# xdslproject/ExaHyPE

Hardware: AMD Instinct MI355X
Metric: DoF-updates/sec, 3D Euler p=5 fused STP+volume+Riemann, 1/2/4/8 MI355X (higher is better)
Workload: dtype f64

## Files before the change

### exahype_amd/csrc/dg_inst.hip

```cpp
#include <cstdarg>
#include <cstdio>
#include "exa_dg_kernels.hpp"
#include "exa_dg_boundary.hpp"
#if EXA_DIM == 2
#include "exa_dg_fused.hpp"
#endif
#if EXA_DIM == 3
#include <algorithm>
#include <vector>
#include "exa_dg_reg.hpp"
#include "exa_dg_stream.hpp"
#include "exa_dg_m8.hpp"
#endif
#include "exa_launch.hpp"

#ifndef EXA_DIM
#error "compile with -DEXA_DIM=2|3 -DEXA_PDE_ID=0|1|2"
#endif

namespace exa {

#if EXA_PDE_ID >= 100
}
#include EXA_USER_PDE_HEADER
// ... 386 lines not shown
    void* step = static_cast<char*>(ops->dev) + StageA<DIM, N, PDE, cpb_of(N)>::STEP_OFF;
    hipLaunchKernelGGL((dg_step_ops_kernel<N>), dim3(1), dim3(64), 0, s, static_cast<const DgOps<N>*>(ops->dev), static_cast<DgStepOps<N>*>(step), dt);
    return step;
}

template <int N>
static int launch_a(const double* u_in, double* u_out, double* trace, long ncells, const CellBox* box, double dt,
                    const double* idx, int n_it, const DgOpsHost* ops, hipStream_t s, const RegFuse* fuse = nullptr) {
    if (box->nbox <= 0) return 0;
    const StageAChoice choice = stage_a_kind<N>(n_it, ops->stage_a_variant, fuse != nullptr);
    [[maybe_unused]] char* img = static_cast<char*>(ops->dev);
    [[maybe_unused]] hipError_t e = hipSuccess;
    switch (choice.kind) {
    case StageAKind::Refused:
        set_error("%s", choice.why);
        return -1;
    case StageAKind::Plain:
        if constexpr (has_plain<N>()) {
            using SP = StagePlain<DIM, N, PDE>;
            auto pk = dg_stage_a_plain_kernel<DIM, N, PDE>;
            static KernelSetup st;
            if (int rc = kernel_setup(st, reinterpret_cast<const void*>(pk), SP::LDS_BYTES, "stage_a", "plain")) return rc;
            hipLaunchKernelGGL(pk, dim3((unsigned)box->nbox), dim3(SP::NT), SP::LDS_BYTES, s, u_in, u_out, trace, ncells, *box, dt, idx[0], idx[1],
                               idx[2], n_it, pack_ops<N>(ops), plain_geo(ops, idx));
            e = hipGetLastError();
            if (e != hipSuccess) { set_error("stage_a (plain) launch (N %d): %s", N, hipGetErrorString(e)); return -2; }
            return 0;
        }
        break;
#if EXA_DIM == 3
    case StageAKind::M8:
        if constexpr (has_m8<N>()) {
            using SM = StageAM8<PDE>;
            auto mk = dg_stage_a_m8_kernel<PDE>;
            static KernelSetup st;
            if (int rc = kernel_setup(st, reinterpret_cast<const void*>(mk), SM::LDS_BYTES, "stage_a", "m8")) return rc;
            const long mwant = box->nbox < SCRATCH_BLOCKS ? box->nbox : SCRATCH_BLOCKS;
            const long mgrid = mwant - ops->stage_a_reserve > 1 ? mwant - ops->stage_a_reserve : 1;
            const void* step = enqueue_step_ops<N>(ops, dt, s);
            hipLaunchKernelGGL(mk, dim3((unsigned)mgrid), dim3(SM::NT), SM::LDS_BYTES, s, u_in, u_out, trace, ncells, *box, dt,
                               idx[0], idx[1], idx[2], n_it, ops->dev, step, reinterpret_cast<const int*>(img + OpsImage<N>::M8_TAB_OFF), plain_geo(ops, idx));
            e = hipGetLastError();
            if (e != hipSuccess) { set_error("stage_a (m8) launch: %s", hipGetErrorString(e)); return -2; }
            return 0;
        }
        break;
    case StageAKind::Stream:
        if constexpr (has_stream<N>()) {
            if (!ops->scratch) { set_error("stage_a: slab missing for N = %d", N); return -1; }
            using SS = StageAStream<N, PDE, 1, 1>;
            auto sk = dg_stage_a_stream_kernel<N, PDE, 1, 1>;
            static KernelSetup st;
            if (int rc = kernel_setup(st, reinterpret_cast<const void*>(sk), SS::LDS_BYTES, "stage_a", "stream")) return rc;
            const long grid = box->nbox < SCRATCH_BLOCKS ? box->nbox : SCRATCH_BLOCKS;
            hipLaunchKernelGGL(sk, dim3((unsigned)grid), dim3(SS::NT), SS::LDS_BYTES, s, u_in, u_out, trace, ncells, *box, dt,
                               idx[0], idx[1], idx[2], n_it, ops->dev, static_cast<double*>(ops->scratch));
            e = hipGetLastError();
            if (e != hipSuccess) { set_error("stage_a (stream) launch (N %d): %s", N, hipGetErrorString(e)); return -2; }
            return 0;
        }
        break;
    case StageAKind::Reg:
        if constexpr (has_reg<N>() && !needs_scratch<N>()) {
            constexpr int CPW = EXA_REG_CPW;
            using SR = StageAReg<N, PDE, CPW>;
            auto rk = dg_stage_a_reg_kernel<N, PDE, CPW, false>;
            if constexpr (!PDE_XT_NCP) {
                if (fuse) rk = dg_stage_a_reg_kernel<N, PDE, CPW, true>;
            }
            static KernelSetup st[2];
            long resident = 0;
            if (int rc = kernel_setup(st[fuse ? 1 : 0], reinterpret_cast<const void*>(rk), SR::LDS_BYTES, "stage_a", "reg", SR::NT * CPW, &resident)) return rc;
            const long rgrid = persistent_grid((box->nbox + CPW - 1) / CPW, resident, ops->stage_a_reserve);
            const void* step = enqueue_step_ops<N>(ops, dt, s);
            hipLaunchKernelGGL(rk, dim3((unsigned)rgrid), dim3(SR::NT * CPW), SR::LDS_BYTES, s, u_in, u_out, trace, ncells, *box, dt,
                               idx[0], idx[1], idx[2], n_it, ops->dev, reinterpret_cast<const int*>(img + OpsImage<N>::REG_TAB_OFF),
                               step, fuse ? *fuse : RegFuse{}, plain_geo(ops, idx));
            e = hipGetLastError();
            if (e != hipSuccess) { set_error("stage_a (reg) launch (N %d): %s", N, hipGetErrorString(e)); return -2; }
            return 0;
        }
        break;
#else
    case StageAKind::M8: case StageAKind::Stream: case StageAKind::Reg: break;
#endif
    case StageAKind::Single:
        if constexpr (!needs_scratch<N>()) {
            constexpr int NT1 = 256;
            constexpr int NNc = ipow(N, DIM);
            constexpr int CPB1 = (NT1 / NNc) > 0 ? NT1 / NNc : 1;
            const long nb1 = (box->nbox + CPB1 - 1) / CPB1;
            hipLaunchKernelGGL((dg_stage_a_single_kernel<DIM, N, PDE, CPB1, NT1>), dim3((unsigned)nb1), dim3(NT1), 0, s, u_in, u_out,
                               trace, ncells, *box, dt, idx[0], idx[1], idx[2], ops->dev);
            e = hipGetLastError();
            if (e != hipSuccess) { set_error("stage_a (single stage) launch (dim %d, N %d): %s", DIM, N, hipGetErrorString(e)); return -2; }
            return 0;
        }
        break;
    case StageAKind::Lds:
        if constexpr (!needs_scratch<N>()) {
            constexpr int CPB = cpb_of(N);
            using SA = StageA<DIM, N, PDE, CPB>;
            auto kern = dg_stage_a_kernel<DIM, N, PDE, CPB>;
            static KernelSetup st;
            long resident = 0;
            if (int rc = kernel_setup(st, reinterpret_cast<const void*>(kern), SA::LDS_BYTES, "stage_a", "", SA::NT, &resident)) return rc;
            const long grid = persistent_grid((box->nbox + CPB - 1) / CPB, resident, ops->stage_a_reserve);
            enqueue_step_ops<N>(ops, dt, s);
            hipLaunchKernelGGL(kern, dim3((unsigned)grid), dim3(SA::NT), SA::LDS_BYTES, s, u_in, u_out, trace, ncells, *box, dt,
                               idx[0], idx[1], idx[2], n_it, ops->dev);
            e = hipGetLastError();
            if (e != hipSuccess) { set_error("stage_a launch (dim %d, N %d): %s", DIM, N, hipGetErrorString(e)); return -2; }
            return 0;
        }
        break;
    }
    set_error("stage_a: the kernel selected for dim %d, N = %d (kind %d) is not built", DIM, N, (int)choice.kind);
    return -1;
}

template <int N> static size_t scratch_bytes_n() {
#if EXA_DIM == 3
    if constexpr (has_stream<N>()) return (size_t)SCRATCH_BLOCKS * StageAStream<N, PDE, 1, 1>::SLAB_D * sizeof(double);
#endif
    return 0;
}

#endif

template <int N>
static int launch_b(double* u, const double* trace, const StageBBox* box, long ncells, double dt, const double* idx,
                    const DgOpsHost* ops, hipStream_t s) {
    constexpr int NFc = ipow(N, DIM - 1);
    constexpr bool SHUFFLE = pow2ceil(NFc) == NFc && !PDE_XT_NCP;
    constexpr int PER = 2 * DIM * (SHUFFLE ? pow2ceil(NFc) : NFc);
    constexpr int CPB = PER >= 256 ? 1 : 256 / PER;
    constexpr int NT_B = SHUFFLE ? ((CPB * PER + 63) / 64) * 64 : 256;
    StageBArgs A;
    long nbox = 1;
    for (int d = 0; d < 3; d++) {
        A.nc[d] = box->nc[d];
        A.lo[d] = box->lo[d];
        A.nb[d] = box->nb[d];
        nbox *= box->nb[d];
    }
    for (int f = 0; f < 6; f++) A.ghost[f] = box->ghost[f];
    A.lam = box->lam;
    if (A.lam && pde_has_xt<PDE>::value) { set_error("stage B with the CFL scan: term sets whose eigenvalues see x, t take the scan with coordinates (exa_pde_eval_device_at)"); return -1; }
    if (nbox <= 0) return 0;
    {
        constexpr int TE = 1 << EXA_STAGE_B_TILE_SHIFT;
        A.tiled = DIM == 3 && box->nb[0] % TE == 0 && box->nb[1] % TE == 0 && box->nb[2] % TE == 0;
    }
    const long nblocks = (nbox + CPB - 1) / CPB;
    if constexpr (!pde_has_xt<PDE>::value) {
        if (A.lam) {
            if constexpr (SHUFFLE)
                hipLaunchKernelGGL((dg_stage_b_kernel<DIM, N, PDE, CPB, NT_B, true>), dim3((unsigned)nblocks), dim3(NT_B), 0, s, u, trace, A,
                                   ncells, nbox, dt, idx[0], idx[1], idx[2], pack_ops<N>(ops));
            else
                hipLaunchKernelGGL((dg_stage_b_dense_kernel<DIM, N, PDE, CPB, NT_B, true>), dim3((unsigned)nblocks), dim3(NT_B), 0, s, u, trace,
                                   A, ncells, nbox, dt, idx[0], idx[1], idx[2], pack_ops<N>(ops), plain_geo(ops, idx));
            hipError_t ec = hipGetLastError();
            if (ec != hipSuccess) { set_error("stage_b (cfl) launch (dim %d, N %d): %s", DIM, N, hipGetErrorString(ec)); return -2; }
            return 0;
        }
    }
    if constexpr (SHUFFLE)
        hipLaunchKernelGGL((dg_stage_b_kernel<DIM, N, PDE, CPB, NT_B>), dim3((unsigned)nblocks), dim3(NT_B), 0, s, u, trace, A,
                           ncells, nbox, dt, idx[0], idx[1], idx[2], pack_ops<N>(ops));
    else
        hipLaunchKernelGGL((dg_stage_b_dense_kernel<DIM, N, PDE, CPB, NT_B>), dim3((unsigned)nblocks), dim3(NT_B), 0, s, u, trace,
                           A, ncells, nbox, dt, idx[0], idx[1], idx[2], pack_ops<N>(ops), plain_geo(ops, idx));
    hipError_t e = hipGetLastError();
    if (e != hipSuccess) {
        set_error("stage_b launch (dim %d, N %d): %s", DIM, N, hipGetErrorString(e));
        return -2;
    }
    return 0;
}

#define EXA_N_CASES(X) X(2) X(3) X(4) X(5) X(6)
#define EXA_N_CASES_HI(X) X(7) X(8)

#ifndef EXA_UNIT_B
static int stage_a(int N, const double* u_in, double* u_out, double* trace, long ncells, const CellBox* box, double dt,
                   const double* idx, int n_it, const DgOpsHost* ops, hipStream_t s) {
    switch (N) {
#define X(n) case n: return launch_a<n>(u_in, u_out, trace, ncells, box, dt, idx, n_it, ops, s);
        EXA_N_CASES(X)
        EXA_N_CASES_HI(X)
#undef X
    }
    set_error("ADER-DG stage A: N = %d is not built for dim %d (supported 2..%d)", N, DIM, MAX_N);
    return -1;
}

static int stage_ba(int N, double* u, const double* trace_in, double* trace_out, long ncells, const CellBox* box, const double* const* ghost,
                    double dt_prev, double dt, const double* idx, int n_it, const DgOpsHost* ops, double* u_plain, hipStream_t s) {
#if EXA_DIM == 3
    RegFuse fz;
    fz.trace_in = trace_in;
    for (int f = 0; f < 6; f++) fz.ghost[f] = ghost ? ghost[f] : nullptr;
    fz.dt_prev = dt_prev;
    fz.u_plain = u_plain;
    if (N == 6) return launch_a<6>(u, u, trace_out, ncells, box, dt, idx, n_it, ops, s, &fz);
#endif
    set_error("the one-kernel step is built for 3-D, N = 6 (got dim %d, N %d)", DIM, N);
    return -1;
}
static int has_stage_ba(int N, int n_it, int variant) { return N == 6 && stage_a_kind<6>(n_it, variant, true).kind == StageAKind::Reg; }

#endif

#define EXA_CAT3_(a, b, c) a##b##_##c
#define EXA_CAT3(a, b, c) EXA_CAT3_(a, b, c)
#if defined(EXA_UNIT_A)
int EXA_CAT3(dg_stage_b_unit_, EXA_DIM, EXA_PDE_ID)(int N, double* u, const double* trace, const StageBBox* box, long ncells, double dt,
                                                    const double* idx, const DgOpsHost* ops, hipStream_t s);
static int stage_b(int N, double* u, const double* trace, const StageBBox* box, long ncells, double dt,
                   const double* idx, const DgOpsHost* ops, hipStream_t s) {
    return EXA_CAT3(dg_stage_b_unit_, EXA_DIM, EXA_PDE_ID)(N, u, trace, box, ncells, dt, idx, ops, s);
}
#else
#if defined(EXA_UNIT_B)
int EXA_CAT3(dg_stage_b_unit_, EXA_DIM, EXA_PDE_ID)(int N, double* u, const double* trace, const StageBBox* box, long ncells, double dt,
                                                    const double* idx, const DgOpsHost* ops, hipStream_t s) {
#else
static int stage_b(int N, double* u, const double* trace, const StageBBox* box, long ncells, double dt,
                   const double* idx, const DgOpsHost* ops, hipStream_t s) {
#endif
    switch (N) {
#define X(n) case n: return launch_b<n>(u, trace, box, ncells, dt, idx, ops, s);
        EXA_N_CASES(X)
        EXA_N_CASES_HI(X)
#undef X
    }
    set_error("ADER-DG stage B: N = %d is not built for dim %d (supported 2..%d)", N, DIM, MAX_N);
    return -1;
}
#endif

#ifndef EXA_UNIT_B

static size_t ops_image(int N, const DgOpsHost* h, void* dst) {
    switch (N) {
#define X(n) case n: if (dst) fill_ops<n>(h, dst); return OpsImage<n>::BYTES;
        EXA_N_CASES(X)
        EXA_N_CASES_HI(X)
#undef X
    }
    return 0;
}

template <int N> static const char* stage_a_name_n(int n_it, int variant) {
    static char buf[96];
    const char* pde = EXA_PDE_ID == 0 ? "exa::EulerRef2D" : (EXA_PDE_ID == 1 ? "exa::Euler" : (EXA_PDE_ID == 2 ? "exa::Advection<1>" : "exa::UserPDE"));
    buf[0] = 0;
    switch (stage_a_kind<N>(n_it, variant, false).kind) {
    case StageAKind::Refused: break;
    case StageAKind::Plain: snprintf(buf, sizeof(buf), "dg_stage_a_plain_kernel<%d, %d, %s>", DIM, N, pde); break;
    case StageAKind::M8: snprintf(buf, sizeof(buf), "dg_stage_a_m8_kernel<%s>", pde); break;
    case StageAKind::Stream: snprintf(buf, sizeof(buf), "dg_stage_a_stream_kernel<%d, %s, 1, 1>", N, pde); break;
    case StageAKind::Single: snprintf(buf, sizeof(buf), "dg_stage_a_single_kernel<%d, %d, %s>", DIM, N, pde); break;
    case StageAKind::Reg: snprintf(buf, sizeof(buf), "dg_stage_a_reg_kernel<%d, %s, %d, false>", N, pde, EXA_REG_CPW); break;
    case StageAKind::Lds: snprintf(buf, sizeof(buf), "dg_stage_a_kernel<%d, %d, %s, %d>", DIM, N, pde, cpb_of(N)); break;
    }
    return buf;
}
static const char* stage_a_name(int N, int n_it, int variant) {
    switch (N) {
#define X(n) case n: return stage_a_name_n<n>(n_it, variant);
        EXA_N_CASES(X)
        EXA_N_CASES_HI(X)
#undef X
    }
    return "";
}

static size_t scratch_bytes(int N) {
    switch (N) {
#define X(n) case n: return scratch_bytes_n<n>();
        EXA_N_CASES(X)
        EXA_N_CASES_HI(X)
#undef X
    }
    return 0;
}

#if EXA_DIM == 2
template <int N>
static int launch_fused(const double* u_in, double* u_out, const long* nc, double dt, const double* idx, const DgOpsHost* ops,
                        hipStream_t s) {
    constexpr int T = FusedTile<N>::T;
    using FU = FusedSingle<N, PDE, T, T>;
    auto kern = dg_fused_single_kernel<N, PDE, T, T>;
    static_assert(FU::LDS_BYTES + sizeof(long) * FU::LC <= 160 * 1024, "fused single-stage step: the tile image does not fit the LDS");
    static KernelSetup st;
    if (int rc = kernel_setup(st, reinterpret_cast<const void*>(kern), FU::LDS_BYTES, "fused step", "")) return rc;
    const long tiles_x = (nc[0] + T - 1) / T, tiles_y = (nc[1] + T - 1) / T;
    hipLaunchKernelGGL(kern, dim3((unsigned)(tiles_x * tiles_y)), dim3(FU::NT), FU::LDS_BYTES, s, u_in, u_out, nc[0], nc[1], tiles_y,
                       dt, idx[0], idx[1], ops->dev);
    hipError_t e = hipGetLastError();
    if (e != hipSuccess) { set_error("fused step launch (N %d): %s", N, hipGetErrorString(e)); return -2; }
    return 0;
}
// ... 104 lines not shown
```

### exahype_amd/csrc/exa_dg_kernels.hpp

```cpp
#pragma once
#include <hip/hip_runtime.h>
#include <type_traits>
#include "exa_dg_common.hpp"
#include "exa_pde.hpp"
#include "exa_dg_plain.hpp"

namespace exa {

__device__ inline long xcd_contiguous(long b, long n) {
    const long per = n / 8;
    return b < per * 8 ? (b % 8) * per + b / 8 : b;
}

template <int I, int E, class F> __device__ inline void static_for(F&& f) {
    if constexpr (I < E) {
        f(std::integral_constant<int, I>{});
        static_for<I + 1, E>(f);
    }
}

#define EXA_AS4 __attribute__((address_space(4)))
template <int N> __device__ inline const EXA_AS4 DgOps<N>* ops_here(const void* raw) {
    unsigned long long a = reinterpret_cast<unsigned long long>(raw);
    asm volatile("" : "+s"(a));
// ... 774 lines not shown
                    tr[(0 * NV + v) * NF + t] = qR;
                    tr[(1 * NV + v) * NF + t] = FR;
                }
            }
        }
    });
    __syncthreads();
    EXA_STAMP(8);

    for (int task = tid; task < CPB * NN * NV; task += NT) {
        const int c = task / (NN * NV), e = task - c * (NN * NV);
        const int n = e / NV, v = e - n * NV;
        const int off = c * CS + G::node_off(n) + v * NTS * SL;
        double us = EXA_LD(off + 2 * ASZ);
#pragma unroll
        for (int d = 0; d < DIM; d++) us += EXA_LD(off + (1 + d) * SL);
        const long cell = cell_id[c];
        if (cell >= 0) u_out[cell * (NN * NV) + e] = us;
    }
    EXA_STAMP(9);
    __syncthreads();
#pragma unroll
    for (int vv = 0; vv < NVA; vv++) um[vv] = unm[vv];
    }
    EXA_STAMP_FLUSH();
}

template <int DIM, int N, class PDE, int CPB, int NT>
__global__ void __launch_bounds__(NT)
dg_stage_a_single_kernel(const double* __restrict__ u_in, double* __restrict__ u_out, double* __restrict__ trace,
                         long ncells, CellBox box, double dt, double idx0, double idx1, double idx2,
                         const void* __restrict__ ops_raw) {
    using G = Geo<DIM, N>;
    constexpr int NV = PDE::NV, NA = PDE::NAUX;
    constexpr int NN = G::NN, NF = G::NF, SL = G::SL;
    constexpr int CS = (1 + DIM) * NV * SL;
    constexpr int KMAX = (CPB * NN + NT - 1) / NT;
    __shared__ __attribute__((aligned(16))) double lds[CPB * CS];
    __shared__ long cell_id[CPB];
    const int tid = threadIdx.x;
    const long b0 = (long)blockIdx.x * CPB;
    const double idx[3] = {idx0, idx1, idx2};
    if (tid < CPB) cell_id[tid] = box.cell(b0 + tid);
    __syncthreads();

    double ur[KMAX][NV];
#pragma unroll
    for (int k = 0; k < KMAX; k++) {
        const int task = tid + k * NT;
        if (task < CPB * NN) {
            const int c = task / NN, n = task - c * NN;
            const long cell = cell_id[c];
            const int off = c * CS + G::node_off(n);
            double a[nz(NA)], F[NV];
#pragma unroll
            for (int v = 0; v < NV; v++) ur[k][v] = cell >= 0 ? u_in[(cell * NN + n) * NV + v] : 1.0;
            PDE::aux_fast(ur[k], a);
#pragma unroll
            for (int v = 0; v < NV; v++) lds[off + v * SL] = ur[k][v];
            static_for<0, DIM>([&](auto dc) {
                constexpr int D = decltype(dc)::value;
                PDE::template flux<D>(ur[k], a, F);
#pragma unroll
                for (int v = 0; v < NV; v++) lds[off + ((1 + D) * NV + v) * SL] = F[v];
            });
        }
    }
    __syncthreads();
    {
        const EXA_AS4 DgOps<N>* o = ops_here<N>(ops_raw);
        for (int task = tid; task < CPB * DIM * NV * NF; task += NT) {
            const int c = task / (DIM * NV * NF);
            int r = task - c * (DIM * NV * NF);
            const int d = r / (NV * NF);
            r -= d * (NV * NF);
            const int v = r / NF, t = r - v * NF;
            const int ps = G::pstride(d);
            const int off = c * CS + G::pbase(d, t);
            double qb[N], Fb[N];
#pragma unroll
            for (int j = 0; j < N; j++) {
                qb[j] = lds[off + v * SL + j * ps];
                Fb[j] = lds[off + ((1 + d) * NV + v) * SL + j * ps];
            }
            const double sc = dt * idx[d];
#pragma unroll
            for (int i = 0; i < N; i++) {
                double sv = 0.0;
#pragma unroll
                for (int j = 0; j < N; j++) sv += o->Kxi[i * N + j] * Fb[j];
                lds[off + ((1 + d) * NV + v) * SL + i * ps] = sc * o->iw[i] * sv;
            }
            double qL = 0.0, qR = 0.0, FL = 0.0, FR = 0.0;
#pragma unroll
            for (int j = 0; j < N; j++) {
                qL += o->phiL[j] * qb[j];
                qR += o->phiR[j] * qb[j];
                FL += o->phiL[j] * Fb[j];
                FR += o->phiR[j] * Fb[j];
            }
            const long cell = cell_id[c];
            if (cell >= 0) {
                double* tl = trace + (((long)d * 2 + 0) * ncells + cell) * (2 * NV * NF);
                double* tr = trace + (((long)d * 2 + 1) * ncells + cell) * (2 * NV * NF);
                tl[(0 * NV + v) * NF + t] = qL;
                tl[(1 * NV + v) * NF + t] = FL;
                tr[(0 * NV + v) * NF + t] = qR;
                tr[(1 * NV + v) * NF + t] = FR;
            }
        }
    }
    __syncthreads();
#pragma unroll
    for (int k = 0; k < KMAX; k++) {
        const int task = tid + k * NT;
        if (task < CPB * NN) {
            const int c = task / NN, n = task - c * NN;
            const long cell = cell_id[c];
            const int off = c * CS + G::node_off(n);
            if (cell >= 0) {
                [[maybe_unused]] double Sq[NV];
                if constexpr (pde_has_source<PDE>::value) PDE::source(ur[k], Sq);
#pragma unroll
                for (int v = 0; v < NV; v++) {
                    double us = ur[k][v];
                    if constexpr (pde_has_source<PDE>::value) us += dt * Sq[v];
#pragma unroll
                    for (int d = 0; d < DIM; d++) us += lds[off + ((1 + d) * NV + v) * SL];
                    u_out[(cell * NN + n) * NV + v] = us;
                }
            }
        }
    }
}

template <int DIM, int N> __device__ inline void face_node_coords(const PlainGeo& g, const long* cc, int d, int side, int y, double* x) {
    int tr[2] = {0, 0};
    if constexpr (DIM == 3) { tr[0] = y / N; tr[1] = y % N; }
    else tr[0] = y;
    int k = 0;
#pragma unroll
    for (int a = 0; a < 3; a++) {
        if (a >= DIM) x[a] = 0.0;
        else if (a == d) x[a] = g.x0[a] + (double)(cc[a] + side) * g.h[a];
        else { x[a] = g.x0[a] + ((double)cc[a] + g.xi[tr[k]]) * g.h[a]; k++; }
    }
}

struct StageBArgs {
    long nc[3];
    long lo[3], nb[3];
    const double* ghost[6];
    int tiled;
    double* lam;
};

template <int DIM, class PDE, int CPB, int NN, int NT>
__device__ inline void stage_b_cfl_scan(const double* unode, long b0, long nbox, double* lam) {
    constexpr int NV = PDE::NV;
    const int tid = threadIdx.x;
    double m = 0.0;
    for (int nd = tid; nd < CPB * NN; nd += NT) {
        if (b0 + nd / NN >= nbox) continue;
        double q[NV];
#pragma unroll
        for (int v = 0; v < NV; v++) q[v] = unode[nd * NV + v];
#pragma unroll
        for (int d = 0; d < DIM; d++) m = nan_max(m, PDE::maxeig(q, d));
    }
#pragma unroll
    for (int o = 32; o > 0; o >>= 1) m = nan_max(m, __shfl_xor(m, o, 64));
    if ((tid & 63) == 0) {
        unsigned long long* lb = reinterpret_cast<unsigned long long*>(lam);
        const unsigned long long mine = (unsigned long long)__double_as_longlong(m);
        if (mine > __hip_atomic_load(lb, __ATOMIC_RELAXED, __HIP_MEMORY_SCOPE_AGENT)) atomicMax(lb, mine);
    }
}
#ifndef EXA_STAGE_B_TILE_SHIFT
#define EXA_STAGE_B_TILE_SHIFT 3
#endif

__host__ __device__ constexpr int pow2ceil(int x) { int p = 1; while (p < x) p <<= 1; return p; }

template <int DIM, int N, class PDE, int CPB, int NT, bool CFL = false>
__global__ void __launch_bounds__(NT)
dg_stage_b_kernel(double* __restrict__ u, const double* __restrict__ trace, StageBArgs A, long ncells, long nbox,
                  double dt, double idx0, double idx1, double idx2, DgOps<N> ops) {
    using G = Geo<DIM, N>;
    constexpr int NV = PDE::NV;
    constexpr int NN = G::NN, NF = G::NF;
    __shared__ double unode[CFL ? CPB * NN * NV : 1];
    constexpr int NFACE = 2 * DIM;
    constexpr int TS = 2 * NV * NF;
    constexpr int GS = pow2ceil(NF);
    static_assert(GS <= 64, "a face must fit one wavefront");
    constexpr int FPB = NT / GS;
    constexpr int NFC = CPB * NFACE;
    constexpr int KB = (NFC + FPB - 1) / FPB;
    __shared__ double fs[CPB * NFACE * NF * NV];
    __shared__ double cL[DIM][N], cR[DIM][N];

    const int tid = threadIdx.x;
    const long b0 = xcd_contiguous(blockIdx.x, gridDim.x) * CPB;
    const double idx[3] = {idx0, idx1, idx2};
#pragma unroll
    for (int i = 0; i < N; i++) {
        if (tid == i) {
#pragma unroll
            for (int d = 0; d < DIM; d++) {
                cL[d][i] = dt * idx[d] * ops.iw[i] * ops.phiL[i];
                cR[d][i] = dt * idx[d] * ops.iw[i] * ops.phiR[i];
            }
        }
    }

    auto cell_of = [&](int c, long* cc) -> long {
        long b = b0 + c;
        if (b >= nbox) b = nbox - 1;
        long cz = 0, cy, cx;
        if (DIM == 3 && A.tiled) {
            constexpr int TSH = EXA_STAGE_B_TILE_SHIFT, TM = (1 << TSH) - 1;
            const long t = b >> (3 * TSH);
            const int w = (int)(b & ((1 << (3 * TSH)) - 1));
            const long tz = A.nb[2] >> TSH, ty = A.nb[1] >> TSH;
            cz = ((t % tz) << TSH) + (w & TM);
            cy = (((t / tz) % ty) << TSH) + ((w >> TSH) & TM);
            cx = ((t / (tz * ty)) << TSH) + (w >> (2 * TSH));
        } else {
            if constexpr (DIM == 3) {
                cz = b % A.nb[2];
                b /= A.nb[2];
            }
            cy = b % A.nb[1];
            cx = b / A.nb[1];
        }
        cc[0] = A.lo[0] + cx;
        cc[1] = A.lo[1] + cy;
        cc[2] = (DIM == 3) ? A.lo[2] + cz : 0;
        return (cc[0] * A.nc[1] + cc[1]) * A.nc[2] + cc[2];
    };

    const int seg = tid / GS, y = tid - seg * GS;
#pragma unroll
    for (int k = 0; k < KB; k++) {
        const int face = seg + k * FPB;
        const bool ok = face < NFC && y < NF;
        double qm[NV], qp[NV], Fm[NV], Fp[NV];
        double lam = 0.0;
        int d = 0;
        if (ok) {
            const int c = face / NFACE, f = face - c * NFACE;
            d = f >> 1;
            const int side = f & 1;
            long cc[3];
            const long cell = cell_of(c, cc);
            long cst[3];
            cst[2] = 1;
            cst[1] = A.nc[2];
            cst[0] = A.nc[1] * A.nc[2];
            long tcell;
            if constexpr (DIM == 3) tcell = d == 0 ? cc[1] * A.nc[2] + cc[2] : (d == 1 ? cc[0] * A.nc[2] + cc[2] : cc[0] * A.nc[1] + cc[1]);
            else tcell = d == 0 ? cc[1] : cc[0];
            const double *pm, *pp;
            if (side == 0) {
                pp = trace + (((long)d * 2 + 0) * ncells + cell) * TS;
                if (cc[d] > 0) pm = trace + (((long)d * 2 + 1) * ncells + cell - cst[d]) * TS;
                else if (A.ghost[d * 2 + 0]) pm = A.ghost[d * 2 + 0] + tcell * TS;
                else pm = trace + (((long)d * 2 + 1) * ncells + cell + (A.nc[d] - 1) * cst[d]) * TS;
            } else {
                pm = trace + (((long)d * 2 + 1) * ncells + cell) * TS;
                if (cc[d] < A.nc[d] - 1) pp = trace + (((long)d * 2 + 0) * ncells + cell + cst[d]) * TS;
                else if (A.ghost[d * 2 + 1]) pp = A.ghost[d * 2 + 1] + tcell * TS;
                else pp = trace + (((long)d * 2 + 0) * ncells + cell - (A.nc[d] - 1) * cst[d]) * TS;
            }
#pragma unroll
            for (int v = 0; v < NV; v++) {
                qm[v] = pm[v * NF + y];
                qp[v] = pp[v * NF + y];
                Fm[v] = pm[(NV + v) * NF + y];
                Fp[v] = pp[(NV + v) * NF + y];
            }
            lam = fmax(PDE::maxeig(qm, d), PDE::maxeig(qp, d));
        }
#pragma unroll
        for (int o = GS / 2; o > 0; o >>= 1) lam = fmax(lam, __shfl_xor(lam, o, GS));
        if (ok) {
#pragma unroll
            for (int v = 0; v < NV; v++)
                fs[(face * NF + y) * NV + v] = 0.5 * (Fm[v] + Fp[v]) - 0.5 * lam * (qp[v] - qm[v]);
        }
    }
    __syncthreads();
    for (int task = tid; task < CPB * NN * NV; task += NT) {
        const int c = task / (NN * NV), e = task - c * (NN * NV);
        if (b0 + c >= nbox) continue;
        const int n = e / NV, v = e - n * NV;
        long cc[3];
        const long cell = cell_of(c, cc);
        double un = u[cell * (NN * NV) + e];
#pragma unroll
        for (int d = 0; d < DIM; d++) {
            const int i = G::coord(n, d), yy = G::face_index(n, d);
            const double fR = fs[((c * NFACE + d * 2 + 1) * NF + yy) * NV + v];
            const double fL = fs[((c * NFACE + d * 2 + 0) * NF + yy) * NV + v];
            un -= cR[d][i] * fR - cL[d][i] * fL;
        }
        u[cell * (NN * NV) + e] = un;
        if constexpr (CFL) unode[task] = un;
    }
    if constexpr (CFL) {
        __syncthreads();
        stage_b_cfl_scan<DIM, PDE, CPB, NN, NT>(unode, b0, nbox, A.lam);
    }
}

template <int DIM, int N, class PDE, int CPB, int NT, bool CFL = false>
__global__ void __launch_bounds__(NT)
dg_stage_b_dense_kernel(double* __restrict__ u, const double* __restrict__ trace, StageBArgs A, long ncells, long nbox,
                  double dt, double idx0, double idx1, double idx2, DgOps<N> ops, PlainGeo geo) {
    using G = Geo<DIM, N>;
    constexpr int NV = PDE::NV;
    constexpr int NN = G::NN, NF = G::NF;
    __shared__ double unode[CFL ? CPB * NN * NV : 1];
    constexpr int NFACE = 2 * DIM;
    constexpr int TS = 2 * NV * NF;
    constexpr int KB = (CPB * NFACE * NF + NT - 1) / NT;
    __shared__ double lam[CPB * NFACE * NF];
    __shared__ double fs[CPB * NFACE * NF * NV];
    __shared__ double cL[DIM][N], cR[DIM][N];

    const int tid = threadIdx.x;
    const long b0 = xcd_contiguous(blockIdx.x, gridDim.x) * CPB;
    const double idx[3] = {idx0, idx1, idx2};
#pragma unroll
    for (int i = 0; i < N; i++) {
        if (tid == i) {
#pragma unroll
            for (int d = 0; d < DIM; d++) {
                cL[d][i] = dt * idx[d] * ops.iw[i] * ops.phiL[i];
                cR[d][i] = dt * idx[d] * ops.iw[i] * ops.phiR[i];
            }
        }
    }

    auto cell_of = [&](int c, long* cc) -> long {
        long b = b0 + c;
        if (b >= nbox) b = nbox - 1;
        long cz = 0, cy, cx;
        if (DIM == 3 && A.tiled) {
            constexpr int TSH = EXA_STAGE_B_TILE_SHIFT, TM = (1 << TSH) - 1;
            const long t = b >> (3 * TSH);
            const int w = (int)(b & ((1 << (3 * TSH)) - 1));
            const long tz = A.nb[2] >> TSH, ty = A.nb[1] >> TSH;
            cz = ((t % tz) << TSH) + (w & TM);
            cy = (((t / tz) % ty) << TSH) + ((w >> TSH) & TM);
            cx = ((t / (tz * ty)) << TSH) + (w >> (2 * TSH));
        } else {
            if constexpr (DIM == 3) {
                cz = b % A.nb[2];
                b /= A.nb[2];
            }
            cy = b % A.nb[1];
            cx = b / A.nb[1];
        }
        cc[0] = A.lo[0] + cx;
        cc[1] = A.lo[1] + cy;
        cc[2] = (DIM == 3) ? A.lo[2] + cz : 0;
        return (cc[0] * A.nc[1] + cc[1]) * A.nc[2] + cc[2];
    };

    double qm[KB][NV], qp[KB][NV], Fm[KB][NV], Fp[KB][NV];
#pragma unroll
    for (int k = 0; k < KB; k++) {
        const int task = tid + k * NT;
        if (task < CPB * NFACE * NF) {
            const int c = task / (NFACE * NF);
            int r = task - c * (NFACE * NF);
            const int f = r / NF, y = r - f * NF;
            const int d = f >> 1, face = f & 1;
            long cc[3];
            const long cell = cell_of(c, cc);
            long cst[3];
            cst[2] = 1;
            cst[1] = A.nc[2];
            cst[0] = A.nc[1] * A.nc[2];
            long tcell;
            if constexpr (DIM == 3) tcell = d == 0 ? cc[1] * A.nc[2] + cc[2] : (d == 1 ? cc[0] * A.nc[2] + cc[2] : cc[0] * A.nc[1] + cc[1]);
            else tcell = d == 0 ? cc[1] : cc[0];
            const double *pm, *pp;
            if (face == 0) {
                pp = trace + (((long)d * 2 + 0) * ncells + cell) * TS;
                if (cc[d] > 0) pm = trace + (((long)d * 2 + 1) * ncells + cell - cst[d]) * TS;
                else if (A.ghost[d * 2 + 0]) pm = A.ghost[d * 2 + 0] + tcell * TS;
                else pm = trace + (((long)d * 2 + 1) * ncells + cell + (A.nc[d] - 1) * cst[d]) * TS;
            } else {
                pm = trace + (((long)d * 2 + 1) * ncells + cell) * TS;
                if (cc[d] < A.nc[d] - 1) pp = trace + (((long)d * 2 + 0) * ncells + cell + cst[d]) * TS;
                else if (A.ghost[d * 2 + 1]) pp = A.ghost[d * 2 + 1] + tcell * TS;
                else pp = trace + (((long)d * 2 + 0) * ncells + cell - (A.nc[d] - 1) * cst[d]) * TS;
            }
#pragma unroll
            for (int v = 0; v < NV; v++) {
                qm[k][v] = pm[v * NF + y];
                qp[k][v] = pp[v * NF + y];
                Fm[k][v] = pm[(NV + v) * NF + y];
                Fp[k][v] = pp[(NV + v) * NF + y];
            }
            if constexpr (pde_has_xt<PDE>::value) {
                double xf[3];
                face_node_coords<DIM, N>(geo, cc, d, face, y, xf);
                lam[task] = fmax(PDE::maxeig_xt(qm[k], xf, geo.t + 0.5 * dt, d), PDE::maxeig_xt(qp[k], xf, geo.t + 0.5 * dt, d));
            } else {
                lam[task] = fmax(PDE::maxeig(qm[k], d), PDE::maxeig(qp[k], d));
            }
        }
    }
    __syncthreads();
#pragma unroll
    for (int k = 0; k < KB; k++) {
        const int task = tid + k * NT;
        if (task < CPB * NFACE * NF) {
            const int face0 = (task / NF) * NF;
            double s = 0.0;
            for (int y = 0; y < NF; y++) s = fmax(s, lam[face0 + y]);
#pragma unroll
            for (int v = 0; v < NV; v++)
                fs[task * NV + v] = 0.5 * (Fm[k][v] + Fp[k][v]) - 0.5 * s * (qp[k][v] - qm[k][v]);
            if constexpr (pde_has_ncp<PDE>::value) {
                const int c = task / (NFACE * NF), r = task - c * (NFACE * NF), f = r / NF, y = r - f * NF;
                const int d = f >> 1, face = f & 1;
                double qa[NV], dq[NV], Dj[NV], xf[3] = {0.0, 0.0, 0.0};
#pragma unroll
                for (int v = 0; v < NV; v++) {
                    qa[v] = 0.5 * (qm[k][v] + qp[k][v]);
                    dq[v] = qp[k][v] - qm[k][v];
                    Dj[v] = 0.0;
                }
                if constexpr (pde_has_xt<PDE>::value) {
                    long cc[3];
                    cell_of(c, cc);
                    face_node_coords<DIM, N>(geo, cc, d, face, y, xf);
                }
                fv_ncp<PDE>(qa, dq, xf, geo.t + 0.5 * dt, d, Dj);
#pragma unroll
                for (int v = 0; v < NV; v++) fs[task * NV + v] += (face == 1 ? 0.5 : -0.5) * Dj[v];
            }
        }
    }
    __syncthreads();
    for (int task = tid; task < CPB * NN * NV; task += NT) {
        const int c = task / (NN * NV), e = task - c * (NN * NV);
        if (b0 + c >= nbox) continue;
        const int n = e / NV, v = e - n * NV;
        long cc[3];
        const long cell = cell_of(c, cc);
        double un = u[cell * (NN * NV) + e];
#pragma unroll
        for (int d = 0; d < DIM; d++) {
            const int i = G::coord(n, d), y = G::face_index(n, d);
            const double fR = fs[((c * NFACE + d * 2 + 1) * NF + y) * NV + v];
            const double fL = fs[((c * NFACE + d * 2 + 0) * NF + y) * NV + v];
            un -= cR[d][i] * fR - cL[d][i] * fL;
        }
        u[cell * (NN * NV) + e] = un;
        if constexpr (CFL) unode[task] = un;
    }
    if constexpr (CFL) {
        __syncthreads();
        stage_b_cfl_scan<DIM, PDE, CPB, NN, NT>(unode, b0, nbox, A.lam);
    }
}

template <int DIM, class PDE>
__global__ void dg_maxeig_kernel(const double* __restrict__ u, long nnodes, double* __restrict__ out) {
    constexpr int NV = PDE::NV;
    double m = 0.0;
    for (long i = blockIdx.x * (long)blockDim.x + threadIdx.x; i < nnodes; i += (long)gridDim.x * blockDim.x) {
        double q[NV];
#pragma unroll
        for (int v = 0; v < NV; v++) q[v] = u[i * NV + v];
#pragma unroll
        for (int d = 0; d < DIM; d++) m = nan_max(m, PDE::maxeig(q, d));
    }
#pragma unroll
    for (int o = 32; o > 0; o >>= 1) m = nan_max(m, __shfl_xor(m, o, 64));
    __shared__ double wm[16];
    if ((threadIdx.x & 63) == 0) wm[threadIdx.x >> 6] = m;
    __syncthreads();
    if (threadIdx.x == 0) {
        for (int w = 1; w < (int)(blockDim.x >> 6); w++) m = nan_max(m, wm[w]);
        atomicMax(reinterpret_cast<unsigned long long*>(out), (unsigned long long)__double_as_longlong(m));
    }
}

}
```

Measured before the change: 13.84 billion.

## Decode stage-B cell addressing once per block and prefetch u before the barrier

```diff
diff --git a/exahype_amd/csrc/dg_inst.hip b/exahype_amd/csrc/dg_inst.hip
--- a/exahype_amd/csrc/dg_inst.hip
+++ b/exahype_amd/csrc/dg_inst.hip
@@ -562,6 +562,7 @@
         constexpr int TE = 1 << EXA_STAGE_B_TILE_SHIFT;
         A.tiled = DIM == 3 && box->nb[0] % TE == 0 && box->nb[1] % TE == 0 && box->nb[2] % TE == 0;
     }
+    A.idx32 = nbox <= 0x7fffffffL;
     const long nblocks = (nbox + CPB - 1) / CPB;
     if constexpr (!pde_has_xt<PDE>::value) {
         if (A.lam) {
diff --git a/exahype_amd/csrc/exa_dg_kernels.hpp b/exahype_amd/csrc/exa_dg_kernels.hpp
--- a/exahype_amd/csrc/exa_dg_kernels.hpp
+++ b/exahype_amd/csrc/exa_dg_kernels.hpp
@@ -950,6 +950,7 @@
     long lo[3], nb[3];
     const double* ghost[6];
     int tiled;
+    int idx32;
     double* lam;
 };
 
@@ -980,6 +981,176 @@
 
 __host__ __device__ constexpr int pow2ceil(int x) { int p = 1; while (p < x) p <<= 1; return p; }
 
+
+template <int DIM, class I> __device__ __forceinline__ void stage_b_slot_coords(const StageBArgs& A, I b, long* cb) {
+    I cz = 0, cy, cx;
+    if (DIM == 3 && A.tiled) {
+        constexpr int TSH = EXA_STAGE_B_TILE_SHIFT, TM = (1 << TSH) - 1;
+        const I t = b >> (3 * TSH);
+        const int w = (int)(b & (I)((1 << (3 * TSH)) - 1));
+        const I tz = (I)(A.nb[2] >> TSH), ty = (I)(A.nb[1] >> TSH);
+        const I tyx = t / tz, tx = tyx / ty;
+        cz = ((t - tyx * tz) << TSH) + (I)(w & TM);
+        cy = ((tyx - tx * ty) << TSH) + (I)((w >> TSH) & TM);
+        cx = (tx << TSH) + (I)(w >> (2 * TSH));
+    } else {
+        I r = b;
+        if constexpr (DIM == 3) {
+            const I q = r / (I)A.nb[2];
+            cz = r - q * (I)A.nb[2];
+            r = q;
+        }
+        cx = r / (I)A.nb[1];
+        cy = r - cx * (I)A.nb[1];
+    }
+    cb[0] = (long)cx;
+    cb[1] = (long)cy;
+    cb[2] = (long)cz;
+}
+
+template <int DIM> struct StageBCell {
+    long cc[3];
+    long cell;
+    const double* pm[2 * DIM];
+    const double* pp[2 * DIM];
+};
+
+template <int DIM, int TS>
+__device__ __forceinline__ void stage_b_decode(const StageBArgs& A, const double* __restrict__ trace, long ncells, long b, long nbox, StageBCell<DIM>& C) {
+    if (b >= nbox) b = nbox - 1;
+    long cb[3];
+    if (A.idx32) stage_b_slot_coords<DIM, unsigned>(A, (unsigned)b, cb);
+    else stage_b_slot_coords<DIM, long>(A, b, cb);
+    C.cc[0] = A.lo[0] + cb[0];
+    C.cc[1] = A.lo[1] + cb[1];
+    C.cc[2] = (DIM == 3) ? A.lo[2] + cb[2] : 0;
+    const long* cc = C.cc;
+    const long cell = (cc[0] * A.nc[1] + cc[1]) * A.nc[2] + cc[2];
+    C.cell = cell;
+    const long cst[3] = {A.nc[1] * A.nc[2], A.nc[2], 1};
+#pragma unroll
+    for (int d = 0; d < DIM; d++) {
+        long tcell;
+        if constexpr (DIM == 3) tcell = d == 0 ? cc[1] * A.nc[2] + cc[2] : (d == 1 ? cc[0] * A.nc[2] + cc[2] : cc[0] * A.nc[1] + cc[1]);
+        else tcell = d == 0 ? cc[1] : cc[0];
+        const double* own_l = trace + (((long)d * 2 + 0) * ncells + cell) * TS;
+        const double* own_r = trace + (((long)d * 2 + 1) * ncells + cell) * TS;
+        C.pp[d * 2] = own_l;
+        if (cc[d] > 0) C.pm[d * 2] = own_r - cst[d] * TS;
+        else if (A.ghost[d * 2 + 0]) C.pm[d * 2] = A.ghost[d * 2 + 0] + tcell * TS;
+        else C.pm[d * 2] = own_r + (A.nc[d] - 1) * cst[d] * TS;
+        C.pm[d * 2 + 1] = own_r;
+        if (cc[d] < A.nc[d] - 1) C.pp[d * 2 + 1] = own_l + cst[d] * TS;
+        else if (A.ghost[d * 2 + 1]) C.pp[d * 2 + 1] = A.ghost[d * 2 + 1] + tcell * TS;
+        else C.pp[d * 2 + 1] = own_l - (A.nc[d] - 1) * cst[d] * TS;
+    }
+}
+
+template <int DIM, int CPB> struct StageBCells {
+    static constexpr int NFACE = 2 * DIM;
+    const StageBCell<DIM>* C;
+    template <int TS>
+    __device__ __forceinline__ void decode(StageBCell<DIM>* table, const StageBArgs& A, const double* __restrict__ trace, long ncells, long b0, long nbox) {
+        if (threadIdx.x < CPB) stage_b_decode<DIM, TS>(A, trace, ncells, b0 + threadIdx.x, nbox, table[threadIdx.x]);
+        __syncthreads();
+        C = table;
+    }
+    __device__ __forceinline__ void pick(int face, const double*& pm, const double*& pp) const {
+        const int c = face / NFACE, f = face - c * NFACE;
+        pm = C[c].pm[f];
+        pp = C[c].pp[f];
+    }
+    __device__ __forceinline__ long cell(int c) const { return C[c].cell; }
+    __device__ __forceinline__ void coords(int c, long* cc) const {
+#pragma unroll
+        for (int a = 0; a < 3; a++) cc[a] = C[c].cc[a];
+    }
+};
+template <int DIM> struct StageBCells<DIM, 1> {
+    static constexpr int NFACE = 2 * DIM;
+    StageBCell<DIM> C;
+    template <int TS>
+    __device__ __forceinline__ void decode(StageBCell<DIM>*, const StageBArgs& A, const double* __restrict__ trace, long ncells, long b0, long nbox) {
+        stage_b_decode<DIM, TS>(A, trace, ncells, b0, nbox, C);
+    }
+    __device__ __forceinline__ void pick(int face, const double*& pm, const double*& pp) const {
+        pm = C.pm[0];
+        pp = C.pp[0];
+#pragma unroll
+        for (int k = 1; k < NFACE; k++) {
+            pm = face == k ? C.pm[k] : pm;
+            pp = face == k ? C.pp[k] : pp;
+        }
+    }
+    __device__ __forceinline__ long cell(int) const { return C.cell; }
+    __device__ __forceinline__ void coords(int, long* cc) const {
+#pragma unroll
+        for (int a = 0; a < 3; a++) cc[a] = C.cc[a];
+    }
+};
+
+template <int DIM, int N>
+__device__ __forceinline__ void stage_b_lift(double (*cL)[N], double (*cR)[N], double dt, double idx0, double idx1, double idx2, const DgOps<N>& ops) {
+    const int tid = threadIdx.x;
+    const int d = tid / N, i = tid - d * N;
+    const double h = d == 0 ? idx0 : (d == 1 || DIM == 2 ? idx1 : idx2);
+    double iw = ops.iw[0], pl = ops.phiL[0], pr = ops.phiR[0];
+#pragma unroll
+    for (int k = 1; k < N; k++) {
+        iw = i == k ? ops.iw[k] : iw;
+        pl = i == k ? ops.phiL[k] : pl;
+        pr = i == k ? ops.phiR[k] : pr;
+    }
+    if (tid < DIM * N) {
+        cL[d][i] = dt * h * iw * pl;
+        cR[d][i] = dt * h * iw * pr;
+    }
+}
+
+template <int DIM, int N, int NV, int CPB, int NT> struct StageBUpdate {
+    using G = Geo<DIM, N>;
+    static constexpr int NN = G::NN, NF = G::NF, NFACE = 2 * DIM, E = G::NN * NV;
+    static constexpr int KU = (CPB * E + NT - 1) / NT;
+
+    static __device__ __forceinline__ bool live(int task, long b0, long nbox, int& c) {
+        c = CPB == 1 ? 0 : task / E;
+        return task < CPB * E && b0 + c < nbox;
+    }
+    static __device__ __forceinline__ long offset(const StageBCells<DIM, CPB>& C, int task, int c) { return C.cell(c) * E + (task - c * E); }
+    static __device__ __forceinline__ void request(const double* u, const StageBCells<DIM, CPB>& C, long b0, long nbox, double (&us)[KU]) {
+        const int tid = threadIdx.x;
+#pragma unroll
+        for (int k = 0; k < KU; k++) {
+            int c;
+            const int task = tid + k * NT;
+            us[k] = live(task, b0, nbox, c) ? u[offset(C, task, c)] : 0.0;
+        }
+    }
+    template <bool CFL>
+    static __device__ __forceinline__ void apply(double* u, const StageBCells<DIM, CPB>& C, long b0, long nbox, const double (&us)[KU], const double* fs,
+                                        const double (*cL)[N], const double (*cR)[N], double* unode) {
+        const int tid = threadIdx.x;
+        __builtin_amdgcn_s_waitcnt(0x0F70);
+#pragma unroll
+        for (int k = 0; k < KU; k++) {
+            int c;
+            const int task = tid + k * NT;
+            if (!live(task, b0, nbox, c)) continue;
+            const int e = task - c * E, n = e / NV, v = e - n * NV;
+            double un = us[k];
+#pragma unroll
+            for (int d = 0; d < DIM; d++) {
+                const int i = G::coord(n, d), y = G::face_index(n, d);
+                const double fR = fs[((c * NFACE + d * 2 + 1) * NF + y) * NV + v];
+                const double fL = fs[((c * NFACE + d * 2 + 0) * NF + y) * NV + v];
+                un -= cR[d][i] * fR - cL[d][i] * fL;
+            }
+            u[offset(C, task, c)] = un;
+            if constexpr (CFL) unode[task] = un;
+        }
+    }
+};
+
 template <int DIM, int N, class PDE, int CPB, int NT, bool CFL = false>
 __global__ void __launch_bounds__(NT)
 dg_stage_b_kernel(double* __restrict__ u, const double* __restrict__ trace, StageBArgs A, long ncells, long nbox,
@@ -987,6 +1158,7 @@
     using G = Geo<DIM, N>;
     constexpr int NV = PDE::NV;
     constexpr int NN = G::NN, NF = G::NF;
+    using U = StageBUpdate<DIM, N, NV, CPB, NT>;
     __shared__ double unode[CFL ? CPB * NN * NV : 1];
     constexpr int NFACE = 2 * DIM;
     constexpr int TS = 2 * NV * NF;
@@ -1000,43 +1172,9 @@
 
     const int tid = threadIdx.x;
     const long b0 = xcd_contiguous(blockIdx.x, gridDim.x) * CPB;
-    const double idx[3] = {idx0, idx1, idx2};
-#pragma unroll
-    for (int i = 0; i < N; i++) {
-        if (tid == i) {
-#pragma unroll
-            for (int d = 0; d < DIM; d++) {
-                cL[d][i] = dt * idx[d] * ops.iw[i] * ops.phiL[i];
-                cR[d][i] = dt * idx[d] * ops.iw[i] * ops.phiR[i];
-            }
-        }
-    }
-
-    auto cell_of = [&](int c, long* cc) -> long {
-        long b = b0 + c;
-        if (b >= nbox) b = nbox - 1;
-        long cz = 0, cy, cx;
-        if (DIM == 3 && A.tiled) {
-            constexpr int TSH = EXA_STAGE_B_TILE_SHIFT, TM = (1 << TSH) - 1;
-            const long t = b >> (3 * TSH);
-            const int w = (int)(b & ((1 << (3 * TSH)) - 1));
-            const long tz = A.nb[2] >> TSH, ty = A.nb[1] >> TSH;
-            cz = ((t % tz) << TSH) + (w & TM);
-            cy = (((t / tz) % ty) << TSH) + ((w >> TSH) & TM);
-            cx = ((t / (tz * ty)) << TSH) + (w >> (2 * TSH));
-        } else {
-            if constexpr (DIM == 3) {
-                cz = b % A.nb[2];
-                b /= A.nb[2];
-            }
-            cy = b % A.nb[1];
-            cx = b / A.nb[1];
-        }
-        cc[0] = A.lo[0] + cx;
-        cc[1] = A.lo[1] + cy;
-        cc[2] = (DIM == 3) ? A.lo[2] + cz : 0;
-        return (cc[0] * A.nc[1] + cc[1]) * A.nc[2] + cc[2];
-    };
+    __shared__ StageBCell<DIM> cell_table[CPB];
+    StageBCells<DIM, CPB> C;
+    C.template decode<TS>(cell_table, A, trace, ncells, b0, nbox);
 
     const int seg = tid / GS, y = tid - seg * GS;
 #pragma unroll
@@ -1045,32 +1183,10 @@
         const bool ok = face < NFC && y < NF;
         double qm[NV], qp[NV], Fm[NV], Fp[NV];
         double lam = 0.0;
-        int d = 0;
         if (ok) {
-            const int c = face / NFACE, f = face - c * NFACE;
-            d = f >> 1;
-            const int side = f & 1;
-            long cc[3];
-            const long cell = cell_of(c, cc);
-            long cst[3];
-            cst[2] = 1;
-            cst[1] = A.nc[2];
-            cst[0] = A.nc[1] * A.nc[2];
-            long tcell;
-            if constexpr (DIM == 3) tcell = d == 0 ? cc[1] * A.nc[2] + cc[2] : (d == 1 ? cc[0] * A.nc[2] + cc[2] : cc[0] * A.nc[1] + cc[1]);
-            else tcell = d == 0 ? cc[1] : cc[0];
+            const int d = (face % NFACE) >> 1;
             const double *pm, *pp;
-            if (side == 0) {
-                pp = trace + (((long)d * 2 + 0) * ncells + cell) * TS;
-                if (cc[d] > 0) pm = trace + (((long)d * 2 + 1) * ncells + cell - cst[d]) * TS;
-                else if (A.ghost[d * 2 + 0]) pm = A.ghost[d * 2 + 0] + tcell * TS;
-                else pm = trace + (((long)d * 2 + 1) * ncells + cell + (A.nc[d] - 1) * cst[d]) * TS;
-            } else {
-                pm = trace + (((long)d * 2 + 1) * ncells + cell) * TS;
-                if (cc[d] < A.nc[d] - 1) pp = trace + (((long)d * 2 + 0) * ncells + cell + cst[d]) * TS;
-                else if (A.ghost[d * 2 + 1]) pp = A.ghost[d * 2 + 1] + tcell * TS;
-                else pp = trace + (((long)d * 2 + 0) * ncells + cell - (A.nc[d] - 1) * cst[d]) * TS;
-            }
+            C.pick(face, pm, pp);
 #pragma unroll
             for (int v = 0; v < NV; v++) {
                 qm[v] = pm[v * NF + y];
@@ -1088,24 +1204,12 @@
                 fs[(face * NF + y) * NV + v] = 0.5 * (Fm[v] + Fp[v]) - 0.5 * lam * (qp[v] - qm[v]);
         }
     }
+    stage_b_lift<DIM, N>(cL, cR, dt, idx0, idx1, idx2, ops);
+    double us[U::KU];
+    __builtin_amdgcn_sched_barrier(0);
+    U::request(u, C, b0, nbox, us);
     __syncthreads();
-    for (int task = tid; task < CPB * NN * NV; task += NT) {
-        const int c = task / (NN * NV), e = task - c * (NN * NV);
-        if (b0 + c >= nbox) continue;
-        const int n = e / NV, v = e - n * NV;
-        long cc[3];
-        const long cell = cell_of(c, cc);
-        double un = u[cell * (NN * NV) + e];
-#pragma unroll
-        for (int d = 0; d < DIM; d++) {
-            const int i = G::coord(n, d), yy = G::face_index(n, d);
-            const double fR = fs[((c * NFACE + d * 2 + 1) * NF + yy) * NV + v];
-            const double fL = fs[((c * NFACE + d * 2 + 0) * NF + yy) * NV + v];
-            un -= cR[d][i] * fR - cL[d][i] * fL;
-        }
-        u[cell * (NN * NV) + e] = un;
-        if constexpr (CFL) unode[task] = un;
-    }
+    U::template apply<CFL>(u, C, b0, nbox, us, fs, cL, cR, unode);
     if constexpr (CFL) {
         __syncthreads();
         stage_b_cfl_scan<DIM, PDE, CPB, NN, NT>(unode, b0, nbox, A.lam);
@@ -1119,6 +1223,7 @@
     using G = Geo<DIM, N>;
     constexpr int NV = PDE::NV;
     constexpr int NN = G::NN, NF = G::NF;
+    using U = StageBUpdate<DIM, N, NV, CPB, NT>;
     __shared__ double unode[CFL ? CPB * NN * NV : 1];
     constexpr int NFACE = 2 * DIM;
     constexpr int TS = 2 * NV * NF;
@@ -1129,74 +1234,22 @@
 
     const int tid = threadIdx.x;
     const long b0 = xcd_contiguous(blockIdx.x, gridDim.x) * CPB;
-    const double idx[3] = {idx0, idx1, idx2};
-#pragma unroll
-    for (int i = 0; i < N; i++) {
-        if (tid == i) {
-#pragma unroll
-            for (int d = 0; d < DIM; d++) {
-                cL[d][i] = dt * idx[d] * ops.iw[i] * ops.phiL[i];
-                cR[d][i] = dt * idx[d] * ops.iw[i] * ops.phiR[i];
-            }
-        }
-    }
-
-    auto cell_of = [&](int c, long* cc) -> long {
-        long b = b0 + c;
-        if (b >= nbox) b = nbox - 1;
-        long cz = 0, cy, cx;
-        if (DIM == 3 && A.tiled) {
-            constexpr int TSH = EXA_STAGE_B_TILE_SHIFT, TM = (1 << TSH) - 1;
-            const long t = b >> (3 * TSH);
-            const int w = (int)(b & ((1 << (3 * TSH)) - 1));
-            const long tz = A.nb[2] >> TSH, ty = A.nb[1] >> TSH;
-            cz = ((t % tz) << TSH) + (w & TM);
-            cy = (((t / tz) % ty) << TSH) + ((w >> TSH) & TM);
-            cx = ((t / (tz * ty)) << TSH) + (w >> (2 * TSH));
-        } else {
-            if constexpr (DIM == 3) {
-                cz = b % A.nb[2];
-                b /= A.nb[2];
-            }
-            cy = b % A.nb[1];
-            cx = b / A.nb[1];
-        }
-        cc[0] = A.lo[0] + cx;
-        cc[1] = A.lo[1] + cy;
-        cc[2] = (DIM == 3) ? A.lo[2] + cz : 0;
-        return (cc[0] * A.nc[1] + cc[1]) * A.nc[2] + cc[2];
-    };
+    __shared__ StageBCell<DIM> cell_table[CPB];
+    StageBCells<DIM, CPB> C;
+    C.template decode<TS>(cell_table, A, trace, ncells, b0, nbox);
 
     double qm[KB][NV], qp[KB][NV], Fm[KB][NV], Fp[KB][NV];
 #pragma unroll
     for (int k = 0; k < KB; k++) {
         const int task = tid + k * NT;
-        if (task < CPB * NFACE * NF) {
-            const int c = task / (NFACE * NF);
-            int r = task - c * (NFACE * NF);
-            const int f = r / NF, y = r - f * NF;
-            const int d = f >> 1, face = f & 1;
-            long cc[3];
-            const long cell = cell_of(c, cc);
-            long cst[3];
-            cst[2] = 1;
-            cst[1] = A.nc[2];
-            cst[0] = A.nc[1] * A.nc[2];
-            long tcell;
-            if constexpr (DIM == 3) tcell = d == 0 ? cc[1] * A.nc[2] + cc[2] : (d == 1 ? cc[0] * A.nc[2] + cc[2] : cc[0] * A.nc[1] + cc[1]);
-            else tcell = d == 0 ? cc[1] : cc[0];
+        const int cf = task / NF;
+        const bool ok = task < CPB * NFACE * NF;
+        double l = 0.0;
+        if (ok) {
+            const int c = cf / NFACE, f = cf - c * NFACE, y = task - cf * NF;
+            const int d = f >> 1;
             const double *pm, *pp;
-            if (face == 0) {
-                pp = trace + (((long)d * 2 + 0) * ncells + cell) * TS;
-                if (cc[d] > 0) pm = trace + (((long)d * 2 + 1) * ncells + cell - cst[d]) * TS;
-                else if (A.ghost[d * 2 + 0]) pm = A.ghost[d * 2 + 0] + tcell * TS;
-                else pm = trace + (((long)d * 2 + 1) * ncells + cell + (A.nc[d] - 1) * cst[d]) * TS;
-            } else {
-                pm = trace + (((long)d * 2 + 1) * ncells + cell) * TS;
-                if (cc[d] < A.nc[d] - 1) pp = trace + (((long)d * 2 + 0) * ncells + cell + cst[d]) * TS;
-                else if (A.ghost[d * 2 + 1]) pp = A.ghost[d * 2 + 1] + tcell * TS;
-                else pp = trace + (((long)d * 2 + 0) * ncells + cell - (A.nc[d] - 1) * cst[d]) * TS;
-            }
+            C.pick(cf, pm, pp);
 #pragma unroll
             for (int v = 0; v < NV; v++) {
                 qm[k][v] = pm[v * NF + y];
@@ -1205,13 +1258,16 @@
                 Fp[k][v] = pp[(NV + v) * NF + y];
             }
             if constexpr (pde_has_xt<PDE>::value) {
+                long cc[3];
                 double xf[3];
-                face_node_coords<DIM, N>(geo, cc, d, face, y, xf);
-                lam[task] = fmax(PDE::maxeig_xt(qm[k], xf, geo.t + 0.5 * dt, d), PDE::maxeig_xt(qp[k], xf, geo.t + 0.5 * dt, d));
+                C.coords(c, cc);
+                face_node_coords<DIM, N>(geo, cc, d, f & 1, y, xf);
+                l = fmax(PDE::maxeig_xt(qm[k], xf, geo.t + 0.5 * dt, d), PDE::maxeig_xt(qp[k], xf, geo.t + 0.5 * dt, d));
             } else {
-                lam[task] = fmax(PDE::maxeig(qm[k], d), PDE::maxeig(qp[k], d));
-            }
-        }
+                l = fmax(PDE::maxeig(qm[k], d), PDE::maxeig(qp[k], d));
+            }
+        }
+        if (ok) lam[task] = l;
     }
     __syncthreads();
 #pragma unroll
@@ -1236,7 +1292,7 @@
                 }
                 if constexpr (pde_has_xt<PDE>::value) {
                     long cc[3];
-                    cell_of(c, cc);
+                    C.coords(c, cc);
                     face_node_coords<DIM, N>(geo, cc, d, face, y, xf);
                 }
                 fv_ncp<PDE>(qa, dq, xf, geo.t + 0.5 * dt, d, Dj);
@@ -1245,29 +1301,18 @@
             }
         }
     }
+    stage_b_lift<DIM, N>(cL, cR, dt, idx0, idx1, idx2, ops);
+    double us[U::KU];
+    __builtin_amdgcn_sched_barrier(0);
+    U::request(u, C, b0, nbox, us);
     __syncthreads();
-    for (int task = tid; task < CPB * NN * NV; task += NT) {
-        const int c = task / (NN * NV), e = task - c * (NN * NV);
-        if (b0 + c >= nbox) continue;
-        const int n = e / NV, v = e - n * NV;
-        long cc[3];
-        const long cell = cell_of(c, cc);
-        double un = u[cell * (NN * NV) + e];
-#pragma unroll
-        for (int d = 0; d < DIM; d++) {
-            const int i = G::coord(n, d), y = G::face_index(n, d);
-            const double fR = fs[((c * NFACE + d * 2 + 1) * NF + y) * NV + v];
-            const double fL = fs[((c * NFACE + d * 2 + 0) * NF + y) * NV + v];
-            un -= cR[d][i] * fR - cL[d][i] * fL;
-        }
-        u[cell * (NN * NV) + e] = un;
-        if constexpr (CFL) unode[task] = un;
-    }
+    U::template apply<CFL>(u, C, b0, nbox, us, fs, cL, cR, unode);
     if constexpr (CFL) {
         __syncthreads();
         stage_b_cfl_scan<DIM, PDE, CPB, NN, NT>(unode, b0, nbox, A.lam);
     }
 }
+
 
 template <int DIM, class PDE>
 __global__ void dg_maxeig_kernel(const double* __restrict__ u, long nnodes, double* __restrict__ out) {
```

New measurement: 13.98 billion (median of 6 runs). 1.01x the previous value.
